# FutureSDR/FutureSDR

Hardware: NVIDIA H100
Metric: Msamples/s (higher is better)
Workload: dtype f32

## Files before the change

### futuresdr_b200/csrc/fir_tc.cu

```cuda
#include <cuda_bf16.h>

#include <algorithm>
#include <climits>
#include <cstdlib>
#include <type_traits>

#include "fir.cuh"

namespace {

constexpr int kStages = 2;
#ifndef B2S_RAW_SLOTS
#define B2S_RAW_SLOTS 6
#endif
constexpr int kRawSlots = B2S_RAW_SLOTS;
constexpr int kRawSlotBytes = 8192;
constexpr int kNumProducerThreads = 256;
constexpr int kNumMathThreads = 256;
constexpr int kNumLoaderThreads = 128;
constexpr int kThreadsTC = kNumMathThreads + kNumProducerThreads + kNumLoaderThreads;
constexpr int kProdWarps = kNumProducerThreads / 32;
constexpr int kMathWarps = kNumMathThreads / 32;
constexpr int kProdWarp0 = kMathWarps;
constexpr int kTmaWarp = kProdWarp0 + kProdWarps;
constexpr int kRegsAtLaunch = 65536 / kThreadsTC / 8 * 8;
constexpr int kMathRegs = 176, kProdRegs = 48, kLoaderRegs = 24;
static_assert(kNumMathThreads * kMathRegs + kNumProducerThreads * kProdRegs + kNumLoaderThreads * kLoaderRegs <=
              kThreadsTC * kRegsAtLaunch, "setmaxnreg budget exceeds the CTA's register allocation");
constexpr int kSchedSlots = 64;
constexpr int kAtomsOut = 16;
constexpr int kMaxDK = 3;
constexpr int kMaxKSteps = (63 + 128 * kMaxDK - 128) / 16 + 1;
constexpr int kSplitBytesMax = (kAtomsOut + kMaxDK - 1) * 1024 * 2;
constexpr int kStageBytes = 2 * kSplitBytesMax;
constexpr int kACores = kMaxDK * 16 + 15;
constexpr int kABytes = kACores * 128;
constexpr int kSmemTC = kStages * kStageBytes + kRawSlots * kRawSlotBytes + 2 * kABytes + 1024  + 256 ;
static_assert(8 * (2 * kStages + 2 * kRawSlots) + 16 + 4 * kStages <= 256, "barriers and tile numbers exceed their 256 bytes");
static_assert(kSmemTC <= 227 * 1024, "tensor FIR shared memory exceeds the 227 KiB per-CTA limit");

enum TcStamp { TL_ENTRY, TL_FIRST_COPY, TL_LAST_COPY, TL_FIRST_FULL, TL_FIRST_STORE, TL_LAST_STORE, TL_CONV_EXIT,
               TL_EXIT, TL_NSTAMPS };
#ifdef B2S_TC_TIMELINE
constexpr int kTlCtas = 1024;
__device__ unsigned long long g_tc_timeline[kTlCtas * TL_NSTAMPS];
#define TC_STAMP(k)                                                                          \
    do {                                                                                     \
        unsigned long long t_;                                                               \
        asm volatile("mov.u64 %0, %%globaltimer;" : "=l"(t_)::"memory");                     \
        if (blockIdx.x < kTlCtas) g_tc_timeline[blockIdx.x * TL_NSTAMPS + (k)] = t_;         \
    } while (0)
#else
#define TC_STAMP(k) do {} while (0)
#endif

__device__ __forceinline__ uint32_t smem_u32(const void *p) { return (uint32_t)__cvta_generic_to_shared(p); }

__device__ __forceinline__ void mbar_init(uint32_t bar, uint32_t count) {
    asm volatile("mbarrier.init.shared::cta.b64 [%0], %1;" ::"r"(bar), "r"(count));
}
__device__ __forceinline__ void mbar_arrive(uint32_t bar) {
    asm volatile("mbarrier.arrive.shared::cta.b64 _, [%0];" ::"r"(bar) : "memory");
}
__device__ __forceinline__ bool mbar_try_wait(uint32_t bar, uint32_t parity) {
    uint32_t ok;
    asm volatile(
        "{\n\t.reg .pred p;\n\t"
        "mbarrier.try_wait.parity.shared::cta.b64 p, [%1], %2;\n\t"
        "selp.b32 %0, 1, 0, p;\n\t}"
        : "=r"(ok) : "r"(bar), "r"(parity) : "memory");
    return ok != 0;
}
__device__ __forceinline__ void mbar_wait(uint32_t bar, uint32_t parity) {
    while (!mbar_try_wait(bar, parity)) {}
}
__device__ __forceinline__ bool elect_one() {
    uint32_t pred;
    asm volatile("{\n\t.reg .pred p;\n\telect.sync _|p, 0xffffffff;\n\tselp.b32 %0, 1, 0, p;\n\t}" : "=r"(pred));
    return pred != 0;
}
__device__ __forceinline__ void fence_barrier_init() { asm volatile("fence.mbarrier_init.release.cluster;" ::: "memory"); }
__device__ __forceinline__ void fence_proxy_async() { asm volatile("fence.proxy.async.shared::cta;" ::: "memory"); }

__device__ __forceinline__ void wgmma_fence() { asm volatile("wgmma.fence.sync.aligned;" ::: "memory"); }
__device__ __forceinline__ void wgmma_commit() { asm volatile("wgmma.commit_group.sync.aligned;" ::: "memory"); }
__device__ __forceinline__ void wgmma_wait_all() { asm volatile("wgmma.wait_group.sync.aligned 0;" ::: "memory"); }
__device__ __forceinline__ void st_global_if(float2 *p, float a, float b, bool pred) {
    asm volatile("{\n\t.reg .pred q;\n\tsetp.ne.b32 q, %3, 0;\n\t@q st.global.v2.f32 [%0], {%1, %2};\n\t}"
                 ::"l"(p), "f"(a), "f"(b), "r"((int)pred) : "memory");
}
__device__ __forceinline__ void st_global_if(float *p, float a, bool pred) {
    asm volatile("{\n\t.reg .pred q;\n\tsetp.ne.b32 q, %2, 0;\n\t@q st.global.f32 [%0], %1;\n\t}"
                 ::"l"(p), "f"(a), "r"((int)pred) : "memory");
}
template <int R> __device__ __forceinline__ void setmaxnreg_inc() { asm volatile("setmaxnreg.inc.sync.aligned.u32 %0;" ::"n"(R)); }
template <int R> __device__ __forceinline__ void setmaxnreg_dec() { asm volatile("setmaxnreg.dec.sync.aligned.u32 %0;" ::"n"(R)); }
__device__ __forceinline__ void wgmma_m64n128(float (&d)[64], uint64_t a_desc, uint64_t b_desc, uint32_t accumulate) {
    asm volatile(
        "{\n\t.reg .pred p;\n\t"
        "setp.ne.b32 p, %66, 0;\n\t"
        "wgmma.mma_async.sync.aligned.m64n128k16.f32.bf16.bf16 "
        "{%0, %1, %2, %3, %4, %5, %6, %7, %8, %9, %10, %11, %12, %13, %14, %15, %16, %17, %18, %19, %20, %21, %22, "
        "%23, %24, %25, %26, %27, %28, %29, %30, %31, %32, %33, %34, %35, %36, %37, %38, %39, %40, %41, %42, %43, "
        "%44, %45, %46, %47, %48, %49, %50, %51, %52, %53, %54, %55, %56, %57, %58, %59, %60, %61, %62, %63}, "
        "%64, %65, p, 1, 1, 0, 0;\n\t}"
        : "+f"(d[0]), "+f"(d[1]), "+f"(d[2]), "+f"(d[3]), "+f"(d[4]), "+f"(d[5]), "+f"(d[6]), "+f"(d[7]),
          "+f"(d[8]), "+f"(d[9]), "+f"(d[10]), "+f"(d[11]), "+f"(d[12]), "+f"(d[13]), "+f"(d[14]), "+f"(d[15]),
          "+f"(d[16]), "+f"(d[17]), "+f"(d[18]), "+f"(d[19]), "+f"(d[20]), "+f"(d[21]), "+f"(d[22]), "+f"(d[23]),
          "+f"(d[24]), "+f"(d[25]), "+f"(d[26]), "+f"(d[27]), "+f"(d[28]), "+f"(d[29]), "+f"(d[30]), "+f"(d[31]),
          "+f"(d[32]), "+f"(d[33]), "+f"(d[34]), "+f"(d[35]), "+f"(d[36]), "+f"(d[37]), "+f"(d[38]), "+f"(d[39]),
          "+f"(d[40]), "+f"(d[41]), "+f"(d[42]), "+f"(d[43]), "+f"(d[44]), "+f"(d[45]), "+f"(d[46]), "+f"(d[47]),
          "+f"(d[48]), "+f"(d[49]), "+f"(d[50]), "+f"(d[51]), "+f"(d[52]), "+f"(d[53]), "+f"(d[54]), "+f"(d[55]),
          "+f"(d[56]), "+f"(d[57]), "+f"(d[58]), "+f"(d[59]), "+f"(d[60]), "+f"(d[61]), "+f"(d[62]), "+f"(d[63])
        : "l"(a_desc), "l"(b_desc), "r"(accumulate)
        : "memory");
}
__device__ __forceinline__ void wgmma_m64n128_rs(float (&d)[64], const uint32_t (&a)[4], uint64_t b_desc,
                                                 uint32_t accumulate) {
    asm volatile(
        "{\n\t.reg .pred p;\n\t"
        "setp.ne.b32 p, %69, 0;\n\t"
        "wgmma.mma_async.sync.aligned.m64n128k16.f32.bf16.bf16 "
        "{%0, %1, %2, %3, %4, %5, %6, %7, %8, %9, %10, %11, %12, %13, %14, %15, %16, %17, %18, %19, %20, %21, %22, "
        "%23, %24, %25, %26, %27, %28, %29, %30, %31, %32, %33, %34, %35, %36, %37, %38, %39, %40, %41, %42, %43, "
        "%44, %45, %46, %47, %48, %49, %50, %51, %52, %53, %54, %55, %56, %57, %58, %59, %60, %61, %62, %63}, "
        "{%64, %65, %66, %67}, %68, p, 1, 1, 0;\n\t}"
        : "+f"(d[0]), "+f"(d[1]), "+f"(d[2]), "+f"(d[3]), "+f"(d[4]), "+f"(d[5]), "+f"(d[6]), "+f"(d[7]),
          "+f"(d[8]), "+f"(d[9]), "+f"(d[10]), "+f"(d[11]), "+f"(d[12]), "+f"(d[13]), "+f"(d[14]), "+f"(d[15]),
          "+f"(d[16]), "+f"(d[17]), "+f"(d[18]), "+f"(d[19]), "+f"(d[20]), "+f"(d[21]), "+f"(d[22]), "+f"(d[23]),
          "+f"(d[24]), "+f"(d[25]), "+f"(d[26]), "+f"(d[27]), "+f"(d[28]), "+f"(d[29]), "+f"(d[30]), "+f"(d[31]),
          "+f"(d[32]), "+f"(d[33]), "+f"(d[34]), "+f"(d[35]), "+f"(d[36]), "+f"(d[37]), "+f"(d[38]), "+f"(d[39]),
          "+f"(d[40]), "+f"(d[41]), "+f"(d[42]), "+f"(d[43]), "+f"(d[44]), "+f"(d[45]), "+f"(d[46]), "+f"(d[47]),
          "+f"(d[48]), "+f"(d[49]), "+f"(d[50]), "+f"(d[51]), "+f"(d[52]), "+f"(d[53]), "+f"(d[54]), "+f"(d[55]),
          "+f"(d[56]), "+f"(d[57]), "+f"(d[58]), "+f"(d[59]), "+f"(d[60]), "+f"(d[61]), "+f"(d[62]), "+f"(d[63])
        : "r"(a[0]), "r"(a[1]), "r"(a[2]), "r"(a[3]), "l"(b_desc), "r"(accumulate)
        : "memory");
}
__device__ __forceinline__ uint32_t ld_shared_b32(uint32_t addr) {
    uint32_t v;
    asm volatile("ld.shared.b32 %0, [%1];" : "=r"(v) : "r"(addr));
    return v;
}

__device__ __forceinline__ uint32_t cvt_bf16x2(float a, float b) {
    uint32_t r;
    asm("cvt.rn.bf16x2.f32 %0, %1, %2;" : "=r"(r) : "f"(b), "f"(a));
    return r;
}
__device__ __forceinline__ void split2(float a, float b, uint32_t &hi, uint32_t &lo) {
    hi = cvt_bf16x2(a, b);
    const float ah = __uint_as_float(hi << 16), bh = __uint_as_float(hi & 0xffff0000u);
    lo = cvt_bf16x2(a - ah, b - bh);
}

__device__ __forceinline__ uint64_t make_desc(uint32_t smem_addr, uint32_t lbo, uint32_t sbo, uint32_t layout) {
    return (uint64_t)((smem_addr & 0x3FFFF) >> 4) | ((uint64_t)(lbo >> 4) << 16) | ((uint64_t)(sbo >> 4) << 32) |
           ((uint64_t)layout << 62);
}
__device__ __forceinline__ uint64_t make_b_desc(uint32_t smem_addr) { return make_desc(smem_addr, 16, 1024, 1); }
__device__ __forceinline__ uint64_t make_a_desc(uint32_t smem_addr) { return make_desc(smem_addr, 128, 128, 0); }

struct TcParams {
    const float *in;
    float *out;
    const float *g;
    long long n_in;
    long long n_out;
    int ntaps;
    int DK;
    int num_tiles;
    int flags;
    int decim;
    const float *hist;
    int hist_items;
    int lead;
    const unsigned *wait_flag;
    unsigned wait_value;
    unsigned *done_flag;
    unsigned done_value;
    unsigned *pub_flag;
    unsigned pub_value;
    unsigned *status;
    unsigned *sched;
};

template <bool COMPLEX>
__global__ void __launch_bounds__(kThreadsTC, 1) fir_tc_kernel(const TcParams prm) {
    extern __shared__ unsigned char smem_raw[];
    const uint32_t raw = smem_u32(smem_raw);
    const uint32_t base = (raw + 1023u) & ~1023u;
    unsigned char *gen_base = smem_raw + (base - raw);
    const uint32_t raw_base = base + kStages * kStageBytes;
    unsigned char *raw_gen = gen_base + kStages * kStageBytes;
    const uint32_t a_base = raw_base + kRawSlots * kRawSlotBytes;
    __nv_bfloat16 *a_gen = reinterpret_cast<__nv_bfloat16 *>(raw_gen + kRawSlots * kRawSlotBytes);
    const uint32_t bar_base = a_base + 2 * kABytes;
    auto full_bar = [&](int s) { return bar_base + 8u * s; };
    auto empty_bar = [&](int s) { return bar_base + 8u * (kStages + s); };
    auto rfull_bar = [&](int r) { return bar_base + 8u * (2 * kStages + r); };
    auto rempty_bar = [&](int r) { return bar_base + 8u * (2 * kStages + kRawSlots + r); };
    const uint32_t tile_ring = bar_base + 8u * (2 * kStages + 2 * kRawSlots);
    const uint32_t stage_tile = tile_ring + 16u;
    volatile int *tile_ring_gen = reinterpret_cast<volatile int *>(gen_base + (tile_ring - base));
    volatile int *stage_tile_gen = reinterpret_cast<volatile int *>(gen_base + (stage_tile - base));

    const int warp = threadIdx.x >> 5, lane = threadIdx.x & 31;
    if (threadIdx.x == 0) TC_STAMP(TL_ENTRY);
    if (prm.pub_flag && blockIdx.x == 0 && threadIdx.x == 0) {
        __threadfence_system();
        asm volatile("st.release.sys.global.u32 [%0], %1;" ::"l"(prm.pub_flag), "r"(prm.pub_value) : "memory");
    }
    const int DK = prm.DK, K = 128 * DK;
    const int atoms = kAtomsOut + DK - 1;
    const int chunk_bytes = atoms * 1024;
    const int split_bytes = 2 * chunk_bytes;
    constexpr int NSEQ = COMPLEX ? 4 : 8;
    constexpr int TILE_BLOCKS = kAtomsOut * NSEQ;
    constexpr long long TILE_ITEMS = (long long)TILE_BLOCKS * 128;

    if (warp == kTmaWarp && lane == 0) {
        for (int s = 0; s < kStages; s++) { mbar_init(full_bar(s), kProdWarps); mbar_init(empty_bar(s), kMathWarps); }
        for (int r = 0; r < kRawSlots; r++) { mbar_init(rfull_bar(r), 1); mbar_init(rempty_bar(r), kProdWarps); }
        fence_barrier_init();
    }
    __syncthreads();

    auto build_strip = [&](auto wait_c) {
        const int a_elems = (K / 8 + 15) * 64;
        for (int i = threadIdx.x; i < a_elems; i += kNumMathThreads + kNumProducerThreads) {
            const int s = i >> 6, r = (i >> 3) & 7, e = i & 7;
            const int t = 8 * s + r + e - 127 - prm.lead;
            const float gv = (t >= 0 && t < prm.ntaps) ? __ldg(prm.g + t) : 0.0f;
            const __nv_bfloat16 hi = __float2bfloat16_rn(gv);
            a_gen[i] = hi;
            a_gen[kABytes / 2 + i] = __float2bfloat16_rn(gv - __bfloat162float(hi));
        }
        fence_proxy_async();
        if constexpr (decltype(wait_c)::value)
            asm volatile("bar.sync 1, %0;" ::"n"(kNumMathThreads + kNumProducerThreads) : "memory");
        else
            asm volatile("bar.arrive 1, %0;" ::"n"(kNumMathThreads + kNumProducerThreads) : "memory");
    };

    constexpr int F4_PER_BLOCK = COMPLEX ? 64 : 32;
    constexpr int BLOCKS_PER_SLOT = 512 / F4_PER_BLOCK;
    constexpr int SLOTS_PER_TILE = (TILE_BLOCKS + kMaxDK - 1 + BLOCKS_PER_SLOT - 1) / BLOCKS_PER_SLOT;
    constexpr int ITEM_BYTES = COMPLEX ? 8 : 4;
    const int in_blocks = TILE_BLOCKS + DK - 1;

    if (warp >= kTmaWarp) {
        setmaxnreg_dec<kLoaderRegs>();
        if (warp != kTmaWarp) return;
        if (elect_one()) {
            int rs = 0;
            uint32_t rphase = 0;
            for (int k = 0;; k++) {
                const int tile = (int)atomicAdd(prm.sched, 1u);
                if (tile >= prm.num_tiles) {
                    mbar_wait(rempty_bar(rs), rphase ^ 1);
                    tile_ring_gen[k & 3] = -1;
                    mbar_arrive(rfull_bar(rs));
                    __threadfence();
                    if (atomicAdd(prm.sched + 1, 1u) == gridDim.x - 1) {
                        __threadfence();
                        atomicExch(prm.sched, 0u);
                        atomicExch(prm.sched + 1, 0u);
                    }
                    break;
                }
                tile_ring_gen[k & 3] = tile;
                const long long item0 = (long long)tile * TILE_ITEMS;
#pragma unroll 1
                for (int s = 0; s < SLOTS_PER_TILE; s++) {
                    const int blk_first = s * BLOCKS_PER_SLOT;
                    if (blk_first >= in_blocks) break;
                    const int nblk = min(BLOCKS_PER_SLOT, in_blocks - blk_first);
                    const long long it0 = item0 + (long long)blk_first * 128;
                    long long items = (long long)nblk * 128;
                    if (it0 + items > prm.n_in) items = prm.n_in - it0;
                    long long bytes = items > 0 ? ((items * ITEM_BYTES) & ~15ll) : 0;
                    mbar_wait(rempty_bar(rs), rphase ^ 1);
                    if (tile == 0 && s == 0 && prm.hist_items > 0) {
                        if (prm.wait_flag) {
                            unsigned long long t0, t1;
                            asm volatile("mov.u64 %0, %%globaltimer;" : "=l"(t0));
                            for (;;) {
                                unsigned v;
                                asm volatile("ld.acquire.sys.global.u32 %0, [%1];" : "=r"(v) : "l"(prm.wait_flag) : "memory");
                                if ((int)(v - prm.wait_value) >= 0) break;
                                asm volatile("mov.u64 %0, %%globaltimer;" : "=l"(t1));
                                if (t1 - t0 > 4000000000ull) { atomicOr(prm.status, 1u); break; }
                                __nanosleep(64);
                            }
                            asm volatile("fence.proxy.async;" ::: "memory");
                        }
                        const uint32_t hb = (uint32_t)prm.hist_items * ITEM_BYTES;
                        const uint32_t rest = bytes > (long long)hb ? (uint32_t)bytes - hb : 0u;
                        asm volatile("mbarrier.arrive.expect_tx.shared::cta.b64 _, [%0], %1;" ::"r"(rfull_bar(rs)), "r"(hb + rest) : "memory");
                        asm volatile("cp.async.bulk.shared::cluster.global.mbarrier::complete_tx::bytes [%0], [%1], %2, [%3];"
                                     ::"r"(raw_base + rs * kRawSlotBytes), "l"(prm.hist), "r"(hb), "r"(rfull_bar(rs)) : "memory");
                        if (rest)
                            asm volatile("cp.async.bulk.shared::cluster.global.mbarrier::complete_tx::bytes [%0], [%1], %2, [%3];"
                                         ::"r"(raw_base + rs * kRawSlotBytes + hb), "l"(prm.in + (COMPLEX ? 2 : 1) * (long long)prm.hist_items),
                                           "r"(rest), "r"(rfull_bar(rs)) : "memory");
                    } else if (bytes > 0) {
                        asm volatile("mbarrier.arrive.expect_tx.shared::cta.b64 _, [%0], %1;" ::"r"(rfull_bar(rs)), "r"((uint32_t)bytes) : "memory");
                        asm volatile("cp.async.bulk.shared::cluster.global.mbarrier::complete_tx::bytes [%0], [%1], %2, [%3];"
                                     ::"r"(raw_base + rs * kRawSlotBytes), "l"(prm.in + (COMPLEX ? 2 : 1) * it0),
                                       "r"((uint32_t)bytes), "r"(rfull_bar(rs)) : "memory");
                    } else {
                        mbar_arrive(rfull_bar(rs));
                    }
                    if (k == 0 && s == 0) TC_STAMP(TL_FIRST_COPY);
                    if (++rs == kRawSlots) { rs = 0; rphase ^= 1; }
                }
            }
            TC_STAMP(TL_LAST_COPY);
        }
        __syncwarp();
    } else if (warp >= kProdWarp0) {
        build_strip(std::false_type{});
        setmaxnreg_dec<kProdRegs>();
        const int tid = threadIdx.x - 32 * kProdWarp0;
        const int fo = tid % F4_PER_BLOCK, rowsel = tid / F4_PER_BLOCK;
        const int kc = COMPLEX ? (fo >> 5) : (fo >> 4);
        const int c16 = COMPLEX ? ((fo & 31) >> 2) : ((fo & 15) >> 1);
        const int wofs = COMPLEX ? (fo & 3) * 4 : (fo & 1) * 8;
        const uint32_t t_off = (uint32_t)(kc * chunk_bytes + wofs + rowsel * 1024);
        uint32_t xj[8];
#pragma unroll
        for (int j = 0; j < 8; j++) xj[j] = (uint32_t)(j * 128 + ((c16 ^ j) << 4));
        const bool alias_thread = rowsel < DK - 1;
        const uint32_t sb = (uint32_t)split_bytes;

        auto convert_tile = [&](auto interior_c, unsigned char *stage_ptr, long long item0, int &rs, uint32_t &rphase) {
            constexpr bool INTERIOR = decltype(interior_c)::value;
            unsigned char *tp = stage_ptr + t_off;
#pragma unroll
            for (int s = 0; s < SLOTS_PER_TILE; s++) {
                if (s * BLOCKS_PER_SLOT >= in_blocks) break;
                mbar_wait(rfull_bar(rs), rphase);
                const float4 *raw = reinterpret_cast<const float4 *>(raw_gen + rs * kRawSlotBytes);
                float4 v[2];
                v[0] = raw[tid];
                v[1] = raw[tid + 256];
                const int rs_cur = rs;
                if (++rs == kRawSlots) { rs = 0; rphase ^= 1; }
                if constexpr (!INTERIOR) {
                    if (s == 0 && item0 == 0 && tid == 0 && prm.done_flag)
                        asm volatile("st.release.sys.global.u32 [%0], %1;" ::"l"(prm.done_flag), "r"(prm.done_value) : "memory");
                }
#pragma unroll
                for (int i = 0; i < 2; i++) {
                    constexpr int ROWS = COMPLEX ? 4 : 8;
                    const int g_ct = COMPLEX ? (8 * (s & 1) + 4 * i) : (8 * i);
                    const int seq = COMPLEX ? (s >> 1) : s;
                    const bool alias_ct = COMPLEX ? ((s & 1) == 0 && i == 0 && s >= 2) : (i == 0 && s >= 1);
                    if (s == SLOTS_PER_TILE - 1) {
                        if (s * BLOCKS_PER_SLOT + rowsel + ROWS * i >= in_blocks) continue;
                    }
                    if (prm.flags & 8) continue;
                    if constexpr (!INTERIOR) {
                        const int bl = s * BLOCKS_PER_SLOT + rowsel + ROWS * i;
                        const long long it = item0 + (long long)bl * 128 + (long long)fo * (COMPLEX ? 2 : 4);
                        const long long gf = it * (COMPLEX ? 2 : 1);
                        const long long total_f = prm.n_in * (COMPLEX ? 2 : 1), copied_f = total_f & ~3ll;
                        float *e = reinterpret_cast<float *>(&v[i]);
                        const long long lead_f = (long long)prm.lead * (COMPLEX ? 2 : 1);
#pragma unroll
                        for (int c = 0; c < 4; c++) {
                            if (gf + c >= total_f || gf + c < lead_f) e[c] = 0.0f;
                            else if (gf + c >= copied_f) e[c] = prm.in[gf + c];
                        }
                    }
                    if constexpr (COMPLEX) {
                        uint32_t rh, rl, ih, il;
                        split2(v[i].x, v[i].z, rh, rl);
                        split2(v[i].y, v[i].w, ih, il);
                        if (seq < NSEQ) {
                            unsigned char *q = tp + g_ct * 1024;
                            *reinterpret_cast<uint32_t *>(q + xj[2 * (seq & 3)]) = rh;
                            *reinterpret_cast<uint32_t *>(q + xj[2 * (seq & 3)] + sb) = rl;
                            *reinterpret_cast<uint32_t *>(q + xj[2 * (seq & 3) + 1]) = ih;
                            *reinterpret_cast<uint32_t *>(q + xj[2 * (seq & 3) + 1] + sb) = il;
                        }
                        if (alias_ct && alias_thread) {
                            unsigned char *q = tp + (g_ct + kAtomsOut) * 1024;
                            *reinterpret_cast<uint32_t *>(q + xj[2 * ((seq - 1) & 3)]) = rh;
                            *reinterpret_cast<uint32_t *>(q + xj[2 * ((seq - 1) & 3)] + sb) = rl;
                            *reinterpret_cast<uint32_t *>(q + xj[2 * ((seq - 1) & 3) + 1]) = ih;
                            *reinterpret_cast<uint32_t *>(q + xj[2 * ((seq - 1) & 3) + 1] + sb) = il;
                        }
                    } else {
                        uint32_t h0, l0, h1, l1;
                        split2(v[i].x, v[i].y, h0, l0);
                        split2(v[i].z, v[i].w, h1, l1);
                        if (seq < NSEQ) {
                            unsigned char *q = tp + g_ct * 1024 + xj[seq & 7];
                            *reinterpret_cast<uint2 *>(q) = make_uint2(h0, h1);
                            *reinterpret_cast<uint2 *>(q + sb) = make_uint2(l0, l1);
                        }
                        if (alias_ct && alias_thread) {
                            unsigned char *q = tp + (g_ct + kAtomsOut) * 1024 + xj[(seq - 1) & 7];
                            *reinterpret_cast<uint2 *>(q) = make_uint2(h0, h1);
                            *reinterpret_cast<uint2 *>(q + sb) = make_uint2(l0, l1);
                        }
                    }
                }
                __syncwarp();
                if (lane == 0) mbar_arrive(rempty_bar(rs_cur));
            }
        };

        int stage = 0, rs = 0;
        uint32_t phase = 0, rphase = 0;
        for (int k = 0;; k++) {
            mbar_wait(rfull_bar(rs), rphase);
            const int tile = tile_ring_gen[k & 3];
            mbar_wait(empty_bar(stage), phase ^ 1);
            if (threadIdx.x == 32 * kProdWarp0) stage_tile_gen[stage] = tile;
            if (tile < 0) {
                __syncwarp();
                if (lane == 0) mbar_arrive(full_bar(stage));
                break;
            }
            const long long item0 = (long long)tile * TILE_ITEMS;
            const bool interior = item0 + (long long)in_blocks * 128 <= prm.n_in &&
                                  !(tile == 0 && (prm.lead | prm.hist_items) != 0);
            unsigned char *stage_ptr = gen_base + stage * kStageBytes;
            if (interior) convert_tile(std::true_type{}, stage_ptr, item0, rs, rphase);
            else convert_tile(std::false_type{}, stage_ptr, item0, rs, rphase);
            fence_proxy_async();
            __syncwarp();
            if (lane == 0) mbar_arrive(full_bar(stage));
            if (++stage == kStages) { stage = 0; phase ^= 1; }
        }
        if (threadIdx.x == 32 * kProdWarp0) TC_STAMP(TL_CONV_EXIT);
    } else {
        build_strip(std::true_type{});
        setmaxnreg_inc<kMathRegs>();
        const int wg = __shfl_sync(0xffffffffu, warp >> 2, 0);
        const int wl = warp & 3, q4 = lane & 3;
        const int D = prm.decim, per_blk = 128 / D;
        const uint32_t a_hi = a_base + 1024u * wg, a_lo = a_hi + kABytes;
        const int p0 = 64 * (1 - wg);
        const int j0 = p0 / 16;
        const int nsteps = (prm.flags & 4) ? 0 : min((p0 + 63 + prm.lead + prm.ntaps - 1) / 16, 8 * DK - 1) - j0 + 1;

        uint32_t ghi[kMaxKSteps][4];
        {
            const uint32_t f0 = a_hi + 256u * (uint32_t)(wl + j0) + 16u * (uint32_t)(lane >> 2) + 4u * (uint32_t)q4;
#pragma unroll
            for (int i = 0; i < kMaxKSteps; i++) {
                const uint32_t f = f0 + 256u * i;
                const bool used = i < nsteps;
                ghi[i][0] = used ? ld_shared_b32(f) : 0u;
                ghi[i][1] = used ? ld_shared_b32(f + 128u) : 0u;
                ghi[i][2] = used ? ld_shared_b32(f + 128u) : 0u;
                ghi[i][3] = used ? ld_shared_b32(f + 256u) : 0u;
            }
        }

        const uint64_t a_lo_desc = make_a_desc(a_lo + 256u * j0);

        int stage = 0;
        uint32_t phase = 0;
        auto mma_tile = [&](float (&acc)[64]) {
            wgmma_fence();
            const uint64_t b_desc = make_b_desc(base + stage * kStageBytes);
#pragma unroll
            for (int i = 0; i < kMaxKSteps; i++) {
                if (i >= nsteps) break;
                const int m = (j0 >> 2) + (i >> 2);
                const uint64_t bh = b_desc + (uint32_t)(((m & 1) * chunk_bytes + (m >> 1) * 1024 + (i & 3) * 32) >> 4);
                wgmma_m64n128_rs(acc, ghi[i], bh, i != 0);
                wgmma_m64n128_rs(acc, ghi[i], bh + (uint32_t)(split_bytes >> 4), 1u);
                wgmma_m64n128(acc, a_lo_desc + 16u * i, bh, 1u);
            }
            wgmma_commit();
        };
        auto release_stage = [&]() {
            wgmma_wait_all();
            __syncwarp();
            if (lane == 0) mbar_arrive(empty_bar(stage));
            if (++stage == kStages) { stage = 0; phase ^= 1; }
        };
        const int log2D = __ffs(D) - 1;
        auto store_tile = [&](const float (&acc)[64], int tile) {
            if (prm.flags & 2) return;
#pragma unroll
            for (int h = 0; h < 2; h++) {
                const int p = 127 - (64 * wg + 16 * wl + (lane >> 2) + 8 * h);
                const int keep = (p & (D - 1)) == D - 1;
                const long long kb = ((long long)tile * TILE_BLOCKS + kAtomsOut * q4 * (COMPLEX ? 1 : 2)) * per_blk +
                                     (p >> log2D);
                const int room = (int)max(min(prm.n_out - kb, (long long)INT_MAX), 0ll) & -keep;
                const int ncols = (int)(((unsigned)room + (unsigned)per_blk - 1u) >> (7 - log2D));
                if constexpr (COMPLEX) {
#pragma unroll
                    for (int gam = 0; gam < 16; gam++)
                        st_global_if(reinterpret_cast<float2 *>(prm.out) + kb + gam * per_blk, acc[4 * gam + 2 * h],
                                     acc[4 * gam + 2 * h + 1], gam < ncols);
                } else {
#pragma unroll
                    for (int n = 0; n < 2 * kAtomsOut; n++)
                        st_global_if(prm.out + (kb + n * per_blk), acc[4 * (n % kAtomsOut) + 2 * h + n / kAtomsOut],
                                     n < ncols);
                }
            }
        };

        float acc[64];
#pragma unroll
        for (int i = 0; i < 64; i++) acc[i] = 0.0f;
        for (int k = 0;; k++) {
            mbar_wait(full_bar(stage), phase);
            const int tile = __shfl_sync(0xffffffffu, stage_tile_gen[stage], 0);
            if (tile < 0) break;
            mma_tile(acc);
            if (threadIdx.x == 0 && k == 0) TC_STAMP(TL_FIRST_FULL);
            release_stage();
            if (threadIdx.x == 0) TC_STAMP(TL_LAST_STORE);
            store_tile(acc, tile);
            if (threadIdx.x == 0 && k == 0) TC_STAMP(TL_FIRST_STORE);
        }
        if (threadIdx.x == 0) TC_STAMP(TL_EXIT);
    }
}

}

bool fir_tc_supported(const b2s_fir *f) {
    if (f->decim == 0 || f->decim > 128 || 128 % f->decim != 0) return false;
    if (f->kind != B2S_C32_F32 && f->kind != B2S_F32_F32) return false;
    return f->ntaps >= 16 && f->ntaps <= 128 * kMaxDK - 127;
}

int32_t fir_tc_prepare(b2s_fir *f) {
    b2s_ctx *ctx = f->ctx;
    if (f->tc_ready) return B2S_OK;
    if (!fir_tc_supported(f)) return b2s_fail(ctx, B2S_EUNSUPPORTED, "tensor FIR: unsupported plan");
    f->tc_kblocks = (int)ceil_div(f->ntaps + 127, 128);
    B2S_CUDA(ctx, cudaFuncSetAttribute(fir_tc_kernel<true>, cudaFuncAttributeMaxDynamicSharedMemorySize, kSmemTC));
    B2S_CUDA(ctx, cudaFuncSetAttribute(fir_tc_kernel<false>, cudaFuncAttributeMaxDynamicSharedMemorySize, kSmemTC));
    for (const void *k : {(const void *)fir_tc_kernel<true>, (const void *)fir_tc_kernel<false>}) {
        cudaFuncAttributes attr;
        B2S_CUDA(ctx, cudaFuncGetAttributes(&attr, k));
        if (attr.numRegs != kRegsAtLaunch)
            return b2s_fail(ctx, B2S_EUNSUPPORTED, "tensor FIR: kernel built with %d registers per thread, its setmaxnreg "
                            "budget assumes %d", attr.numRegs, kRegsAtLaunch);
    }
    if (const char *e = getenv("B2S_TC_FLAGS")) f->tc_flags = atoi(e);
    B2S_TRY(f->d_tc_sched.alloc(ctx, 2 * kSchedSlots, "tensor FIR: tile counters"));
    B2S_CUDA(ctx, cudaMemset(f->d_tc_sched.get(), 0, 2 * kSchedSlots * sizeof(unsigned)));
    f->tc_ready = true;
    return B2S_OK;
}

int32_t fir_tc_launch_hist(b2s_fir *f, const FirHist *h, const void *d_in, size_t n_in, void *d_out, size_t n_out,
                           cudaStream_t stream) {
    b2s_ctx *ctx = f->ctx;
    if (n_out == 0) return B2S_OK;
    if (!f->tc_ready) return b2s_fail(ctx, B2S_ESTATE, "tensor FIR not prepared");
    const bool cplx = f->kind == B2S_C32_F32;
    const size_t item = cplx ? 8 : 4, q = 16 / item;
    const uintptr_t a_in = reinterpret_cast<uintptr_t>(d_in), a_out = reinterpret_cast<uintptr_t>(d_out);
    if ((a_in % item) || (a_out % item)) return B2S_EAGAIN;
    const size_t n_hist = h ? h->n_hist : 0;
    size_t lead;
    if (n_hist) {
        const uintptr_t a_h = reinterpret_cast<uintptr_t>(h->d_hist);
        if ((a_h % item) || (a_in & 15)) return B2S_EAGAIN;
        lead = (a_h / item) % q;
        if ((lead + n_hist) % q) return B2S_EAGAIN;
        if (lead + n_hist > 1024 || n_in * item < 16) return B2S_EAGAIN;
    } else {
        lead = (a_in / item) % q;
    }
    const int DK = (int)ceil_div(f->ntaps + lead + 127, 128);
    if (DK > kMaxDK) return B2S_EAGAIN;
    TcParams prm;
    prm.lead = (int)lead;
    prm.hist_items = n_hist ? (int)(lead + n_hist) : 0;
    prm.hist = n_hist ? (const float *)h->d_hist - lead * (item / 4) : nullptr;
    prm.in = (const float *)d_in - (lead + n_hist) * (item / 4);
    prm.wait_flag = (h && n_hist) ? h->wait_flag : nullptr;
    prm.wait_value = h ? h->wait_value : 0;
    prm.done_flag = (h && n_hist) ? h->done_flag : nullptr;
    prm.done_value = h ? h->done_value : 0;
    prm.pub_flag = h ? h->publish_flag : nullptr;
    prm.pub_value = h ? h->publish_value : 0;
    prm.status = ctx->d_status;
    prm.sched = f->d_tc_sched.get() + 2 * (f->tc_launches++ % kSchedSlots);
    prm.out = (float *)d_out;
    prm.g = f->d_ptaps.get() + (size_t)f->decim * f->Upad;
    prm.n_in = (long long)(lead + n_hist + n_in);
    prm.n_out = (long long)n_out;
    prm.decim = (int)f->decim;
    prm.ntaps = (int)f->ntaps;
    prm.DK = DK;
    const long long tile_items = cplx ? 64 * 128 : 128 * 128;
    prm.num_tiles = (int)ceil_div(n_out * f->decim, (size_t)tile_items);
    prm.flags = f->tc_flags;
    const int grid = std::min(prm.num_tiles, ctx->sm_count);
    if (prm.wait_flag) ctx->flag_ops++;
    if (cplx) fir_tc_kernel<true><<<grid, kThreadsTC, kSmemTC, stream>>>(prm);
    else fir_tc_kernel<false><<<grid, kThreadsTC, kSmemTC, stream>>>(prm);
    B2S_CHECK_LAUNCH(ctx);
    return B2S_OK;
}

#ifdef B2S_TC_TIMELINE
extern "C" int b2s_tc_timeline_read(unsigned long long *host, int ctas) {
    const size_t bytes = sizeof(unsigned long long) * TL_NSTAMPS * (size_t)std::min(std::max(ctas, 0), kTlCtas);
    void *d = nullptr;
    if (cudaGetSymbolAddress(&d, g_tc_timeline) != cudaSuccess) return -1;
    if (cudaMemcpy(host, d, bytes, cudaMemcpyDeviceToHost) != cudaSuccess) return -1;
    if (cudaMemset(d, 0, sizeof(unsigned long long) * TL_NSTAMPS * kTlCtas) != cudaSuccess) return -1;
    return TL_NSTAMPS;
}
#endif

int32_t fir_tc_launch(b2s_fir *f, const void *d_in, size_t n_in, void *d_out, size_t n_out,
                      cudaStream_t stream) {
    const int32_t rc = fir_tc_launch_hist(f, nullptr, d_in, n_in, d_out, n_out, stream);
    if (rc == B2S_EAGAIN) return fir_direct_launch(f, d_in, n_in, d_out, n_out, stream);
    return rc;
}
```

Before: 172,600.

## Schedule FIR work in half-size units with adaptive wide tiles and L2 prefetch

Splits the tensor-core FIR work into half-width units (8 atoms) that are handed out through the atomic scheduler. A CTA claims two units at once as a full-width tile while plenty of work remains, then falls back to single half-units near the end to balance the tail across SMs. The half-width path uses m64n64 wgmma variants and adjusted convert/store indexing. It also issues a bulk L2 prefetch for the second claimed unit's input. The cost is extra scheduler reads, templated code paths that add code size, and less efficient N=64 MMAs on the tail.

```diff
diff --git a/futuresdr_b200/csrc/fir_tc.cu b/futuresdr_b200/csrc/fir_tc.cu
--- a/futuresdr_b200/csrc/fir_tc.cu
+++ b/futuresdr_b200/csrc/fir_tc.cu
@@ -15,6 +15,9 @@
 #endif
 constexpr int kRawSlots = B2S_RAW_SLOTS;
 constexpr int kRawSlotBytes = 8192;
+#ifndef B2S_TC_L2_PREFETCH
+#define B2S_TC_L2_PREFETCH 1
+#endif
 constexpr int kNumProducerThreads = 256;
 constexpr int kNumMathThreads = 256;
 constexpr int kNumLoaderThreads = 128;
@@ -29,6 +32,7 @@
               kThreadsTC * kRegsAtLaunch, "setmaxnreg budget exceeds the CTA's register allocation");
 constexpr int kSchedSlots = 64;
 constexpr int kAtomsOut = 16;
+constexpr int kAtomsHalf = kAtomsOut / 2;
 constexpr int kMaxDK = 3;
 constexpr int kMaxKSteps = (63 + 128 * kMaxDK - 128) / 16 + 1;
 constexpr int kSplitBytesMax = (kAtomsOut + kMaxDK - 1) * 1024 * 2;
@@ -136,6 +140,40 @@
         : "r"(a[0]), "r"(a[1]), "r"(a[2]), "r"(a[3]), "l"(b_desc), "r"(accumulate)
         : "memory");
 }
+__device__ __forceinline__ void wgmma_m64n64(float (&d)[64], uint64_t a_desc, uint64_t b_desc, uint32_t accumulate) {
+    asm volatile(
+        "{\n\t.reg .pred p;\n\t"
+        "setp.ne.b32 p, %34, 0;\n\t"
+        "wgmma.mma_async.sync.aligned.m64n64k16.f32.bf16.bf16 "
+        "{%0, %1, %2, %3, %4, %5, %6, %7, %8, %9, %10, %11, %12, %13, %14, %15, %16, %17, %18, %19, %20, %21, %22, "
+        "%23, %24, %25, %26, %27, %28, %29, %30, %31}, "
+        "%32, %33, p, 1, 1, 0, 0;\n\t}"
+        : "+f"(d[0]), "+f"(d[1]), "+f"(d[2]), "+f"(d[3]), "+f"(d[4]), "+f"(d[5]), "+f"(d[6]), "+f"(d[7]),
+          "+f"(d[8]), "+f"(d[9]), "+f"(d[10]), "+f"(d[11]), "+f"(d[12]), "+f"(d[13]), "+f"(d[14]), "+f"(d[15]),
+          "+f"(d[16]), "+f"(d[17]), "+f"(d[18]), "+f"(d[19]), "+f"(d[20]), "+f"(d[21]), "+f"(d[22]), "+f"(d[23]),
+          "+f"(d[24]), "+f"(d[25]), "+f"(d[26]), "+f"(d[27]), "+f"(d[28]), "+f"(d[29]), "+f"(d[30]), "+f"(d[31])
+        : "l"(a_desc), "l"(b_desc), "r"(accumulate)
+        : "memory");
+}
+__device__ __forceinline__ void wgmma_m64n64_rs(float (&d)[64], const uint32_t (&a)[4], uint64_t b_desc,
+                                                uint32_t accumulate) {
+    asm volatile(
+        "{\n\t.reg .pred p;\n\t"
+        "setp.ne.b32 p, %37, 0;\n\t"
+        "wgmma.mma_async.sync.aligned.m64n64k16.f32.bf16.bf16 "
+        "{%0, %1, %2, %3, %4, %5, %6, %7, %8, %9, %10, %11, %12, %13, %14, %15, %16, %17, %18, %19, %20, %21, %22, "
+        "%23, %24, %25, %26, %27, %28, %29, %30, %31}, "
+        "{%32, %33, %34, %35}, %36, p, 1, 1, 0;\n\t}"
+        : "+f"(d[0]), "+f"(d[1]), "+f"(d[2]), "+f"(d[3]), "+f"(d[4]), "+f"(d[5]), "+f"(d[6]), "+f"(d[7]),
+          "+f"(d[8]), "+f"(d[9]), "+f"(d[10]), "+f"(d[11]), "+f"(d[12]), "+f"(d[13]), "+f"(d[14]), "+f"(d[15]),
+          "+f"(d[16]), "+f"(d[17]), "+f"(d[18]), "+f"(d[19]), "+f"(d[20]), "+f"(d[21]), "+f"(d[22]), "+f"(d[23]),
+          "+f"(d[24]), "+f"(d[25]), "+f"(d[26]), "+f"(d[27]), "+f"(d[28]), "+f"(d[29]), "+f"(d[30]), "+f"(d[31])
+        : "r"(a[0]), "r"(a[1]), "r"(a[2]), "r"(a[3]), "l"(b_desc), "r"(accumulate)
+        : "memory");
+}
+__device__ __forceinline__ void prefetch_l2_bulk(const void *p, uint32_t bytes) {
+    asm volatile("cp.async.bulk.prefetch.L2.global [%0], %1;" ::"l"(p), "r"(bytes) : "memory");
+}
 __device__ __forceinline__ uint32_t ld_shared_b32(uint32_t addr) {
     uint32_t v;
     asm volatile("ld.shared.b32 %0, [%1];" : "=r"(v) : "r"(addr));
@@ -168,7 +206,7 @@
     long long n_out;
     int ntaps;
     int DK;
-    int num_tiles;
+    int num_units;
     int flags;
     int decim;
     const float *hist;
@@ -216,7 +254,8 @@
     const int split_bytes = 2 * chunk_bytes;
     constexpr int NSEQ = COMPLEX ? 4 : 8;
     constexpr int TILE_BLOCKS = kAtomsOut * NSEQ;
-    constexpr long long TILE_ITEMS = (long long)TILE_BLOCKS * 128;
+    constexpr int UNIT_BLOCKS = kAtomsHalf * NSEQ;
+    constexpr long long UNIT_ITEMS = (long long)UNIT_BLOCKS * 128;
 
     if (warp == kTmaWarp && lane == 0) {
         for (int s = 0; s < kStages; s++) { mbar_init(full_bar(s), kProdWarps); mbar_init(empty_bar(s), kMathWarps); }
@@ -245,8 +284,9 @@
     constexpr int F4_PER_BLOCK = COMPLEX ? 64 : 32;
     constexpr int BLOCKS_PER_SLOT = 512 / F4_PER_BLOCK;
     constexpr int SLOTS_PER_TILE = (TILE_BLOCKS + kMaxDK - 1 + BLOCKS_PER_SLOT - 1) / BLOCKS_PER_SLOT;
+    constexpr int SLOTS_PER_UNIT = (UNIT_BLOCKS + kMaxDK - 1 + BLOCKS_PER_SLOT - 1) / BLOCKS_PER_SLOT;
     constexpr int ITEM_BYTES = COMPLEX ? 8 : 4;
-    const int in_blocks = TILE_BLOCKS + DK - 1;
+    auto in_blocks_of = [&](int code) { return ((code & 1) ? TILE_BLOCKS : UNIT_BLOCKS) + DK - 1; };
 
     if (warp >= kTmaWarp) {
         setmaxnreg_dec<kLoaderRegs>();
@@ -254,9 +294,23 @@
         if (elect_one()) {
             int rs = 0;
             uint32_t rphase = 0;
+            auto draw = [&](bool first) {
+                unsigned w = 1;
+                if (!first) {
+                    unsigned c;
+                    asm volatile("ld.relaxed.gpu.global.u32 %0, [%1];" : "=r"(c) : "l"(prm.sched) : "memory");
+                    if ((long long)c + 2ll * gridDim.x < prm.num_units) w = 2;
+                }
+                const int u = (int)atomicAdd(prm.sched, w);
+                if (u >= prm.num_units) return -1;
+                return 2 * u + (w == 2 && u + 1 < prm.num_units ? 1 : 0);
+            };
+            int code = draw(true);
+            const int second = code >= 0 ? draw(false) : -1;
             for (int k = 0;; k++) {
-                const int tile = (int)atomicAdd(prm.sched, 1u);
-                if (tile >= prm.num_tiles) {
+                if (k == 1) code = second;
+                else if (k > 1) code = draw(false);
+                if (code < 0) {
                     mbar_wait(rempty_bar(rs), rphase ^ 1);
                     tile_ring_gen[k & 3] = -1;
                     mbar_arrive(rfull_bar(rs));
@@ -268,8 +322,10 @@
                     }
                     break;
                 }
-                tile_ring_gen[k & 3] = tile;
-                const long long item0 = (long long)tile * TILE_ITEMS;
+                tile_ring_gen[k & 3] = code;
+                const int tile = code >> 1;
+                const int in_blocks = in_blocks_of(code);
+                const long long item0 = (long long)tile * UNIT_ITEMS;
 #pragma unroll 1
                 for (int s = 0; s < SLOTS_PER_TILE; s++) {
                     const int blk_first = s * BLOCKS_PER_SLOT;
@@ -314,6 +370,14 @@
                     if (k == 0 && s == 0) TC_STAMP(TL_FIRST_COPY);
                     if (++rs == kRawSlots) { rs = 0; rphase ^= 1; }
                 }
+#if B2S_TC_L2_PREFETCH
+                if (k == 0 && second >= 0) {
+                    const long long it0 = (long long)(second >> 1) * UNIT_ITEMS;
+                    const long long items = min((long long)in_blocks_of(second) * 128, prm.n_in - it0);
+                    if (items > 0)
+                        prefetch_l2_bulk(prm.in + (COMPLEX ? 2 : 1) * it0, (uint32_t)((items * ITEM_BYTES) & ~15ll));
+                }
+#endif
             }
             TC_STAMP(TL_LAST_COPY);
         }
@@ -333,11 +397,13 @@
         const bool alias_thread = rowsel < DK - 1;
         const uint32_t sb = (uint32_t)split_bytes;
 
-        auto convert_tile = [&](auto interior_c, unsigned char *stage_ptr, long long item0, int &rs, uint32_t &rphase) {
-            constexpr bool INTERIOR = decltype(interior_c)::value;
+        auto convert_tile = [&](auto interior_c, auto wide_c, unsigned char *stage_ptr, long long item0, int in_blocks,
+                                int &rs, uint32_t &rphase) {
+            constexpr bool INTERIOR = decltype(interior_c)::value, WIDE = decltype(wide_c)::value;
+            constexpr int A = WIDE ? kAtomsOut : kAtomsHalf, SLOTS = WIDE ? SLOTS_PER_TILE : SLOTS_PER_UNIT;
             unsigned char *tp = stage_ptr + t_off;
 #pragma unroll
-            for (int s = 0; s < SLOTS_PER_TILE; s++) {
+            for (int s = 0; s < SLOTS; s++) {
                 if (s * BLOCKS_PER_SLOT >= in_blocks) break;
                 mbar_wait(rfull_bar(rs), rphase);
                 const float4 *raw = reinterpret_cast<const float4 *>(raw_gen + rs * kRawSlotBytes);
@@ -353,10 +419,10 @@
 #pragma unroll
                 for (int i = 0; i < 2; i++) {
                     constexpr int ROWS = COMPLEX ? 4 : 8;
-                    const int g_ct = COMPLEX ? (8 * (s & 1) + 4 * i) : (8 * i);
-                    const int seq = COMPLEX ? (s >> 1) : s;
-                    const bool alias_ct = COMPLEX ? ((s & 1) == 0 && i == 0 && s >= 2) : (i == 0 && s >= 1);
-                    if (s == SLOTS_PER_TILE - 1) {
+                    const int g_ct = WIDE ? (COMPLEX ? 8 * (s & 1) + 4 * i : 8 * i) : (COMPLEX ? 4 * i : 0);
+                    const int seq = WIDE ? (COMPLEX ? s >> 1 : s) : (COMPLEX ? s : 2 * s + i);
+                    const bool alias_ct = g_ct == 0 && seq >= 1;
+                    if (s == SLOTS - 1) {
                         if (s * BLOCKS_PER_SLOT + rowsel + ROWS * i >= in_blocks) continue;
                     }
                     if (prm.flags & 8) continue;
@@ -385,7 +451,7 @@
                             *reinterpret_cast<uint32_t *>(q + xj[2 * (seq & 3) + 1] + sb) = il;
                         }
                         if (alias_ct && alias_thread) {
-                            unsigned char *q = tp + (g_ct + kAtomsOut) * 1024;
+                            unsigned char *q = tp + (g_ct + A) * 1024;
                             *reinterpret_cast<uint32_t *>(q + xj[2 * ((seq - 1) & 3)]) = rh;
                             *reinterpret_cast<uint32_t *>(q + xj[2 * ((seq - 1) & 3)] + sb) = rl;
                             *reinterpret_cast<uint32_t *>(q + xj[2 * ((seq - 1) & 3) + 1]) = ih;
@@ -401,7 +467,7 @@
                             *reinterpret_cast<uint2 *>(q + sb) = make_uint2(l0, l1);
                         }
                         if (alias_ct && alias_thread) {
-                            unsigned char *q = tp + (g_ct + kAtomsOut) * 1024 + xj[(seq - 1) & 7];
+                            unsigned char *q = tp + (g_ct + A) * 1024 + xj[(seq - 1) & 7];
                             *reinterpret_cast<uint2 *>(q) = make_uint2(h0, h1);
                             *reinterpret_cast<uint2 *>(q + sb) = make_uint2(l0, l1);
                         }
@@ -416,20 +482,28 @@
         uint32_t phase = 0, rphase = 0;
         for (int k = 0;; k++) {
             mbar_wait(rfull_bar(rs), rphase);
-            const int tile = tile_ring_gen[k & 3];
+            const int code = tile_ring_gen[k & 3];
             mbar_wait(empty_bar(stage), phase ^ 1);
-            if (threadIdx.x == 32 * kProdWarp0) stage_tile_gen[stage] = tile;
-            if (tile < 0) {
+            if (threadIdx.x == 32 * kProdWarp0) stage_tile_gen[stage] = code;
+            if (code < 0) {
                 __syncwarp();
                 if (lane == 0) mbar_arrive(full_bar(stage));
                 break;
             }
-            const long long item0 = (long long)tile * TILE_ITEMS;
+            const long long item0 = (long long)(code >> 1) * UNIT_ITEMS;
+            const int in_blocks = in_blocks_of(code);
             const bool interior = item0 + (long long)in_blocks * 128 <= prm.n_in &&
-                                  !(tile == 0 && (prm.lead | prm.hist_items) != 0);
+                                  !(item0 == 0 && (prm.lead | prm.hist_items) != 0);
             unsigned char *stage_ptr = gen_base + stage * kStageBytes;
-            if (interior) convert_tile(std::true_type{}, stage_ptr, item0, rs, rphase);
-            else convert_tile(std::false_type{}, stage_ptr, item0, rs, rphase);
+            const std::true_type wide{};
+            const std::false_type half{};
+            if (code & 1) {
+                if (interior) convert_tile(std::true_type{}, wide, stage_ptr, item0, in_blocks, rs, rphase);
+                else convert_tile(std::false_type{}, wide, stage_ptr, item0, in_blocks, rs, rphase);
+            } else {
+                if (interior) convert_tile(std::true_type{}, half, stage_ptr, item0, in_blocks, rs, rphase);
+                else convert_tile(std::false_type{}, half, stage_ptr, item0, in_blocks, rs, rphase);
+            }
             fence_proxy_async();
             __syncwarp();
             if (lane == 0) mbar_arrive(full_bar(stage));
@@ -465,7 +539,8 @@
 
         int stage = 0;
         uint32_t phase = 0;
-        auto mma_tile = [&](float (&acc)[64]) {
+        auto mma_tile = [&](auto wide_c, float (&acc)[64]) {
+            constexpr bool WIDE = decltype(wide_c)::value;
             wgmma_fence();
             const uint64_t b_desc = make_b_desc(base + stage * kStageBytes);
 #pragma unroll
@@ -473,9 +548,15 @@
                 if (i >= nsteps) break;
                 const int m = (j0 >> 2) + (i >> 2);
                 const uint64_t bh = b_desc + (uint32_t)(((m & 1) * chunk_bytes + (m >> 1) * 1024 + (i & 3) * 32) >> 4);
-                wgmma_m64n128_rs(acc, ghi[i], bh, i != 0);
-                wgmma_m64n128_rs(acc, ghi[i], bh + (uint32_t)(split_bytes >> 4), 1u);
-                wgmma_m64n128(acc, a_lo_desc + 16u * i, bh, 1u);
+                if constexpr (WIDE) {
+                    wgmma_m64n128_rs(acc, ghi[i], bh, i != 0);
+                    wgmma_m64n128_rs(acc, ghi[i], bh + (uint32_t)(split_bytes >> 4), 1u);
+                    wgmma_m64n128(acc, a_lo_desc + 16u * i, bh, 1u);
+                } else {
+                    wgmma_m64n64_rs(acc, ghi[i], bh, i != 0);
+                    wgmma_m64n64_rs(acc, ghi[i], bh + (uint32_t)(split_bytes >> 4), 1u);
+                    wgmma_m64n64(acc, a_lo_desc + 16u * i, bh, 1u);
+                }
             }
             wgmma_commit();
         };
@@ -486,26 +567,26 @@
             if (++stage == kStages) { stage = 0; phase ^= 1; }
         };
         const int log2D = __ffs(D) - 1;
-        auto store_tile = [&](const float (&acc)[64], int tile) {
+        auto store_tile = [&](auto wide_c, const float (&acc)[64], int unit) {
+            constexpr int A = decltype(wide_c)::value ? kAtomsOut : kAtomsHalf;
             if (prm.flags & 2) return;
 #pragma unroll
             for (int h = 0; h < 2; h++) {
                 const int p = 127 - (64 * wg + 16 * wl + (lane >> 2) + 8 * h);
                 const int keep = (p & (D - 1)) == D - 1;
-                const long long kb = ((long long)tile * TILE_BLOCKS + kAtomsOut * q4 * (COMPLEX ? 1 : 2)) * per_blk +
+                const long long kb = ((long long)unit * UNIT_BLOCKS + A * q4 * (COMPLEX ? 1 : 2)) * per_blk +
                                      (p >> log2D);
                 const int room = (int)max(min(prm.n_out - kb, (long long)INT_MAX), 0ll) & -keep;
                 const int ncols = (int)(((unsigned)room + (unsigned)per_blk - 1u) >> (7 - log2D));
                 if constexpr (COMPLEX) {
 #pragma unroll
-                    for (int gam = 0; gam < 16; gam++)
+                    for (int gam = 0; gam < A; gam++)
                         st_global_if(reinterpret_cast<float2 *>(prm.out) + kb + gam * per_blk, acc[4 * gam + 2 * h],
                                      acc[4 * gam + 2 * h + 1], gam < ncols);
                 } else {
 #pragma unroll
-                    for (int n = 0; n < 2 * kAtomsOut; n++)
-                        st_global_if(prm.out + (kb + n * per_blk), acc[4 * (n % kAtomsOut) + 2 * h + n / kAtomsOut],
-                                     n < ncols);
+                    for (int n = 0; n < 2 * A; n++)
+                        st_global_if(prm.out + (kb + n * per_blk), acc[4 * (n % A) + 2 * h + n / A], n < ncols);
                 }
             }
         };
@@ -513,16 +594,20 @@
         float acc[64];
 #pragma unroll
         for (int i = 0; i < 64; i++) acc[i] = 0.0f;
-        for (int k = 0;; k++) {
-            mbar_wait(full_bar(stage), phase);
-            const int tile = __shfl_sync(0xffffffffu, stage_tile_gen[stage], 0);
-            if (tile < 0) break;
-            mma_tile(acc);
+        auto run_tile = [&](auto wide_c, int unit, int k) {
+            mma_tile(wide_c, acc);
             if (threadIdx.x == 0 && k == 0) TC_STAMP(TL_FIRST_FULL);
             release_stage();
             if (threadIdx.x == 0) TC_STAMP(TL_LAST_STORE);
-            store_tile(acc, tile);
+            store_tile(wide_c, acc, unit);
             if (threadIdx.x == 0 && k == 0) TC_STAMP(TL_FIRST_STORE);
+        };
+        for (int k = 0;; k++) {
+            mbar_wait(full_bar(stage), phase);
+            const int code = __shfl_sync(0xffffffffu, stage_tile_gen[stage], 0);
+            if (code < 0) break;
+            if (code & 1) run_tile(std::true_type{}, code >> 1, k);
+            else run_tile(std::false_type{}, code >> 1, k);
         }
         if (threadIdx.x == 0) TC_STAMP(TL_EXIT);
     }
@@ -599,10 +684,10 @@
     prm.decim = (int)f->decim;
     prm.ntaps = (int)f->ntaps;
     prm.DK = DK;
-    const long long tile_items = cplx ? 64 * 128 : 128 * 128;
-    prm.num_tiles = (int)ceil_div(n_out * f->decim, (size_t)tile_items);
+    const long long unit_items = cplx ? 32 * 128 : 64 * 128;
+    prm.num_units = (int)ceil_div(n_out * f->decim, (size_t)unit_items);
     prm.flags = f->tc_flags;
-    const int grid = std::min(prm.num_tiles, ctx->sm_count);
+    const int grid = std::min(prm.num_units, ctx->sm_count);
     if (prm.wait_flag) ctx->flag_ops++;
     if (cplx) fir_tc_kernel<true><<<grid, kThreadsTC, kSmemTC, stream>>>(prm);
     else fir_tc_kernel<false><<<grid, kThreadsTC, kSmemTC, stream>>>(prm);
```

Result: no change. 171,300, median of 6 (-0.8%).
